# cure-lab/MagicDrive

Hardware: NVIDIA H100
Metric: 6-view 224x400 denoising-steps/sec (higher is better)
Workload: dtype bf16

## Files before the change

### magicdrive_b200/csrc/attention_wgmma.cuh

```cuda
#pragma once
#include "ptx.cuh"
#include "wgmma.cuh"

namespace mdb {

constexpr int ATT_BM = 128;

constexpr int ATT_MAX_SRC = 3;
struct AttnKvMaps {
  CUtensorMap k[ATT_MAX_SRC], v[ATT_MAX_SRC];
};

struct AttnParams {
  __nv_bfloat16* out;
  int ldo;
  int lq, lk;
  const int* kv_index;
  int n_sets;
  int n_src;
  float scale_log2;
  int q_step;
};

template <int D, int BN_ = 0>
struct AttnCfg {
  static constexpr int KD = (D + 63) / 64;
  static constexpr int D16 = (D + 15) / 16 * 16;
  static constexpr int BN = BN_ ? BN_ : ((D16 <= 64) ? 128 : 64);
  static constexpr int TILE_Q = ATT_BM * 128;
  static constexpr int TILE_KV = BN * 128;
  static constexpr int SMEM_Q = KD * TILE_Q;
  static constexpr int STAGES_FIT = (232448 - 1024 - 256 - SMEM_Q) / (2 * KD * TILE_KV);
  static constexpr int STAGES = STAGES_FIT > 4 ? 4 : STAGES_FIT;
  static constexpr int SMEM_KV = STAGES * 2 * KD * TILE_KV;
  static constexpr int kSmemBytes = SMEM_Q + SMEM_KV + 1024 + 256;
  static constexpr int kConsumerWarps = 8;
  static constexpr int kThreads = 32 * kConsumerWarps + 32;
  static constexpr int SACC = BN / 2;
  static constexpr int OACC = D16 / 2;
  static_assert(STAGES >= 1 && kSmemBytes <= 232448, "shared memory");
};

template <int D, int BN_>
__global__ void __launch_bounds__(AttnCfg<D, BN_>::kThreads, 1)
attention_wgmma_kernel(const __grid_constant__ CUtensorMap tmQ, const __grid_constant__ AttnKvMaps kvm, const AttnParams p) {
  using Cfg = AttnCfg<D, BN_>;
  constexpr int KD = Cfg::KD, D16 = Cfg::D16, BN = Cfg::BN, STAGES = Cfg::STAGES;
  constexpr int TILE_Q = Cfg::TILE_Q, TILE_KV = Cfg::TILE_KV;
  extern __shared__ uint8_t smem_raw[];
  uint8_t* smem = reinterpret_cast<uint8_t*>((reinterpret_cast<uintptr_t>(smem_raw) + 1023) & ~uintptr_t(1023));
  uint8_t* smQ = smem;
  uint8_t* smK = smQ + Cfg::SMEM_Q;
  uint8_t* smV = smK + STAGES * KD * TILE_KV;
  uint64_t* bars = reinterpret_cast<uint64_t*>(smV + STAGES * KD * TILE_KV);
  uint64_t* q_full = bars;
  uint64_t* q_empty = bars + 1;
  uint64_t* kv_full = bars + 2;
  uint64_t* kv_empty = bars + 2 + STAGES;

  const int warp = threadIdx.x >> 5, lane = threadIdx.x & 31;
  const int b = blockIdx.z, head = blockIdx.y;
  const int ntiles = (p.lk + BN - 1) / BN;
  const int nq = (p.lq + ATT_BM - 1) / ATT_BM;
  const int q_step = p.q_step > 0 ? p.q_step : nq;
  const int n_own = (nq - static_cast<int>(blockIdx.x) + q_step - 1) / q_step;
  const bool kv_resident = ntiles == 1 && p.n_sets == 1 && n_own > 1;
  auto q0_of = [&](int o) { return (static_cast<int>(blockIdx.x) + o * q_step) * ATT_BM; };

  if (warp == Cfg::kConsumerWarps && lane == 0) {
    prefetch_tmap(&tmQ);
    for (int i = 0; i < p.n_src; ++i) {
      prefetch_tmap(&kvm.k[i]);
      prefetch_tmap(&kvm.v[i]);
    }
    mbar_init(q_full, 1);
    mbar_init(q_empty, Cfg::kConsumerWarps);
    for (int i = 0; i < STAGES; ++i) {
      mbar_init(&kv_full[i], 1);
      mbar_init(&kv_empty[i], Cfg::kConsumerWarps);
    }
    fence_barrier_init();
  }
  __syncthreads();
  asm volatile("griddepcontrol.wait;" ::: "memory");
  asm volatile("griddepcontrol.launch_dependents;" ::: "memory");

  if (warp == Cfg::kConsumerWarps) {
    if (lane == 0) {
      int stage = 0;
      uint32_t phase = 0;
      for (int o = 0; o < n_own; ++o) {
        if (o > 0) mbar_wait(q_empty, static_cast<uint32_t>(o - 1) & 1u);
        mbar_arrive_expect_tx(q_full, KD * TILE_Q);
#pragma unroll
        for (int c = 0; c < KD; ++c) tma_load_4d(&tmQ, q_full, smQ + c * TILE_Q, c * 64, head, q0_of(o), b);
        if (kv_resident && o > 0) continue;
        for (int set = 0; set < p.n_sets; ++set) {
          const int kve = p.kv_index ? p.kv_index[b * p.n_sets + set] : b;
          const int kvb = kve & 0xffffff;
          const CUtensorMap* km = &kvm.k[kve >> 24];
          const CUtensorMap* vm = &kvm.v[kve >> 24];
          for (int j = 0; j < ntiles; ++j) {
            mbar_wait(&kv_empty[stage], phase ^ 1);
            mbar_arrive_expect_tx(&kv_full[stage], 2 * KD * TILE_KV);
#pragma unroll
            for (int c = 0; c < KD; ++c) {
              tma_load_4d(km, &kv_full[stage], smK + (stage * KD + c) * TILE_KV, c * 64, head, j * BN, kvb);
              tma_load_4d(vm, &kv_full[stage], smV + (stage * KD + c) * TILE_KV, c * 64, head, j * BN, kvb);
            }
            if (++stage == STAGES) {
              stage = 0;
              phase ^= 1;
            }
          }
        }
      }
    }
    return;
  }

  const int wg = warp >> 2;
  const int q = lane & 3;
  const int rloc = 64 * wg + 16 * (warp & 3) + (lane >> 2);
  const float sc = p.scale_log2;
  int stage = 0;
  uint32_t phase = 0;
  for (int o = 0; o < n_own; ++o) {
    const int q0 = q0_of(o);
    mbar_wait(q_full, static_cast<uint32_t>(o) & 1u);
    for (int set = 0; set < p.n_sets; ++set) {
      float oacc[Cfg::OACC];
#pragma unroll
      for (int i = 0; i < Cfg::OACC; ++i) oacc[i] = 0.f;
      float m[2] = {-INFINITY, -INFINITY}, l[2] = {0.f, 0.f};
      for (int j = 0; j < ntiles; ++j) {
        const int st = kv_resident ? 0 : stage;
        mbar_wait(&kv_full[st], kv_resident ? 0u : phase);
        float s[Cfg::SACC];
        wgmma_fence();
#pragma unroll
        for (int k = 0; k < D16 / 16; ++k) {
          const int c = k / 4, kk = k % 4;
          const uint64_t adesc = make_sw128_kmajor_desc(smem_u32(smQ + c * TILE_Q + wg * (64 * 128))) + 2 * kk;
          const uint64_t bdesc = make_sw128_kmajor_desc(smem_u32(smK + (st * KD + c) * TILE_KV)) + 2 * kk;
          WgmmaSS<BN>::run(s, adesc, bdesc, k > 0 ? 1u : 0u);
        }
        wgmma_commit();
        wgmma_wait<0>();
        const int kbase = j * BN;
        if (kbase + BN > p.lk) {
#pragma unroll
          for (int g = 0; g < BN / 8; ++g)
#pragma unroll
            for (int e = 0; e < 2; ++e)
              if (kbase + 8 * g + 2 * q + e >= p.lk) s[4 * g + e] = s[4 * g + 2 + e] = -INFINITY;
        }
        float corr[2];
#pragma unroll
        for (int h = 0; h < 2; ++h) {
          float mx = -INFINITY;
#pragma unroll
          for (int g = 0; g < BN / 8; ++g) mx = fmaxf(mx, fmaxf(s[4 * g + 2 * h], s[4 * g + 2 * h + 1]));
          mx = fmaxf(mx, __shfl_xor_sync(0xffffffffu, mx, 1));
          mx = fmaxf(mx, __shfl_xor_sync(0xffffffffu, mx, 2));
          const float m_new = fmaxf(m[h], mx * sc);
          corr[h] = exp2f(m[h] - m_new);
          m[h] = m_new;
        }
        uint32_t pa[BN / 16][4];
        float rs[2] = {0.f, 0.f};
#pragma unroll
        for (int kk = 0; kk < BN / 16; ++kk) {
#pragma unroll
          for (int r = 0; r < 4; ++r) {
            const int h = r & 1;
            const int i0 = 8 * kk + 4 * (r >> 1) + 2 * h;
            const float p0 = exp2f(fmaf(s[i0], sc, -m[h]));
            const float p1 = exp2f(fmaf(s[i0 + 1], sc, -m[h]));
            rs[h] += p0 + p1;
            pa[kk][r] = pack_bf16(p0, p1);
          }
        }
#pragma unroll
        for (int h = 0; h < 2; ++h) l[h] = l[h] * corr[h] + rs[h];
#pragma unroll
        for (int g = 0; g < D16 / 8; ++g) {
          oacc[4 * g] *= corr[0], oacc[4 * g + 1] *= corr[0];
          oacc[4 * g + 2] *= corr[1], oacc[4 * g + 3] *= corr[1];
        }
        wgmma_fence();
#pragma unroll
        for (int kk = 0; kk < BN / 16; ++kk) {
          const uint64_t bdesc = make_sw128_mnmajor_desc(smem_u32(smV + st * KD * TILE_KV), TILE_KV) + (2048u >> 4) * kk;
          WgmmaRSBmn<D16>::run(oacc, pa[kk], bdesc, 1u);
        }
        wgmma_commit();
        wgmma_wait<0>();
        if (!kv_resident) {
          if (lane == 0) mbar_arrive(&kv_empty[stage]);
          if (++stage == STAGES) {
            stage = 0;
            phase ^= 1;
          }
        }
      }
#pragma unroll
      for (int h = 0; h < 2; ++h) {
        l[h] += __shfl_xor_sync(0xffffffffu, l[h], 1);
        l[h] += __shfl_xor_sync(0xffffffffu, l[h], 2);
      }
      const float inv[2] = {1.0f / l[0], 1.0f / l[1]};
#pragma unroll
      for (int h = 0; h < 2; ++h) {
        const int qrow = q0 + rloc + 8 * h;
        if (qrow >= p.lq) continue;
        __nv_bfloat16* orow = p.out + (static_cast<long long>(b) * p.lq + qrow) * p.ldo + head * D;
#pragma unroll
        for (int g = 0; g < D16 / 8; ++g) {
          const int col = 8 * g + 2 * q;
          if (col >= D) continue;
          float f0 = oacc[4 * g + 2 * h] * inv[h], f1 = oacc[4 * g + 2 * h + 1] * inv[h];
          if (set > 0) {
            const float2 pf = __bfloat1622float2(*reinterpret_cast<const __nv_bfloat162*>(orow + col));
            f0 = __bfloat162float(__float2bfloat16_rn(f0)) + pf.x;
            f1 = __bfloat162float(__float2bfloat16_rn(f1)) + pf.y;
          }
          *reinterpret_cast<uint32_t*>(orow + col) = pack_bf16(f0, f1);
        }
      }
    }
    __syncwarp();
    if (lane == 0) mbar_arrive(q_empty);
  }
}

}
```

### magicdrive_b200/csrc/capi_attention.cu

```cuda
#include <cuda_bf16.h>
#include <cuda_runtime.h>

#include <stdlib.h>
#include <string.h>

#include "../../include/magicdrive_b200.h"
#define MDB_NEED_TENSORMAP
#include "common_host.h"
#include "attention_wgmma.cuh"

namespace {

bool make_qkv_map(CUtensorMap* m, const void* ptr, int d, int heads, int l, int b, int ld, int rows) {
  mdb::EncodeTiledFn enc = mdb::get_encode();
  if (!enc) return false;
  cuuint64_t dims[4] = {(cuuint64_t)d, (cuuint64_t)heads, (cuuint64_t)l, (cuuint64_t)b};
  cuuint64_t strides[3] = {(cuuint64_t)d * 2, (cuuint64_t)ld * 2, (cuuint64_t)l * ld * 2};
  cuuint32_t box[4] = {64u, 1u, (cuuint32_t)rows, 1u};
  cuuint32_t estr[4] = {1u, 1u, 1u, 1u};
  return enc(m, CU_TENSOR_MAP_DATA_TYPE_BFLOAT16, 4, const_cast<void*>(ptr), dims, strides, box, estr,
             CU_TENSOR_MAP_INTERLEAVE_NONE, CU_TENSOR_MAP_SWIZZLE_128B, CU_TENSOR_MAP_L2_PROMOTION_L2_256B,
             CU_TENSOR_MAP_FLOAT_OOB_FILL_NONE) == CUDA_SUCCESS;
}

struct KvSources {
  const void* k[mdb::ATT_MAX_SRC];
  const void* v[mdb::ATT_MAX_SRC];
  int ldk[mdb::ATT_MAX_SRC], ldv[mdb::ATT_MAX_SRC], b_kv[mdb::ATT_MAX_SRC];
  int n;
};

bool make_kv_maps(mdb::AttnKvMaps* m, const KvSources& s, int d, int heads, int lk, int rows) {
  for (int i = 0; i < mdb::ATT_MAX_SRC; ++i) {
    const int j = i < s.n ? i : 0;
    if (!make_qkv_map(&m->k[i], s.k[j], d, heads, lk, s.b_kv[j], s.ldk[j], rows) ||
        !make_qkv_map(&m->v[i], s.v[j], d, heads, lk, s.b_kv[j], s.ldv[j], rows))
      return false;
  }
  return true;
}

int attn_num_sms() {
  static int sms = 0;
  if (!sms) {
    int dev = 0;
    cudaGetDevice(&dev);
    if (cudaDeviceGetAttribute(&sms, cudaDevAttrMultiProcessorCount, dev) != cudaSuccess || sms <= 0) sms = 132;
  }
  return sms;
}

int multi_q_step(int b, int heads, int lq, int lk, int n_sets, int bn) {
  if (lk > bn || n_sets != 1) return 0;
  const char* e = getenv("MDB_ATTN_MULTIQ");
  if (e && e[0] == '0') return 0;
  const int nq = (lq + mdb::ATT_BM - 1) / mdb::ATT_BM;
  const long long per_tile_ctas = static_cast<long long>(b) * heads;
  const long long slots = attn_num_sms();
  if (per_tile_ctas * nq <= slots) return 0;
  long long gx = slots / per_tile_ctas;
  if (gx < 1) gx = 1;
  if (gx >= nq) return 0;
  return static_cast<int>(gx);
}

template <int D, int BN_>
int launch_attention(const void* q, int ldq, const KvSources& src, void* out, int ldo, int b, int heads, int lq, int lk,
                     const int* kv_index, int n_sets, float scale, cudaStream_t st) {
  using Cfg = mdb::AttnCfg<D, BN_>;
  static bool attr = false;
  if (!attr) {
    cudaError_t e = cudaFuncSetAttribute(mdb::attention_wgmma_kernel<D, BN_>, cudaFuncAttributeMaxDynamicSharedMemorySize, Cfg::kSmemBytes);
    if (e != cudaSuccess) return mdb::set_error(MDB_ERR_CUDA, "attention_wgmma_kernel smem attr: %s", cudaGetErrorString(e));
    attr = true;
  }
  CUtensorMap tq;
  mdb::AttnKvMaps kvm;
  if (!make_qkv_map(&tq, q, D, heads, lq, b, ldq, mdb::ATT_BM) || !make_kv_maps(&kvm, src, D, heads, lk, Cfg::BN))
    return mdb::set_error(MDB_ERR_CUDA, "mdb_attention: cuTensorMapEncodeTiled failed (d=%d heads=%d lq=%d lk=%d)", D, heads, lq, lk);
  mdb::AttnParams p;
  p.out = static_cast<__nv_bfloat16*>(out);
  p.ldo = ldo, p.lq = lq, p.lk = lk, p.kv_index = kv_index, p.n_sets = n_sets, p.n_src = src.n;
  p.scale_log2 = scale * 1.4426950408889634f;
  p.q_step = multi_q_step(b, heads, lq, lk, n_sets, Cfg::BN);
  dim3 grid(p.q_step > 0 ? p.q_step : (lq + mdb::ATT_BM - 1) / mdb::ATT_BM, heads, b);
  cudaError_t le = mdb::launch_pdl(mdb::attention_wgmma_kernel<D, BN_>, grid, dim3(Cfg::kThreads), Cfg::kSmemBytes, st, tq, kvm, p);
  if (le != cudaSuccess) return mdb::set_error(MDB_ERR_CUDA, "attention_wgmma_kernel launch: %s", cudaGetErrorString(le));
  cudaError_t e2 = cudaGetLastError();
  if (e2 != cudaSuccess) return mdb::set_error(MDB_ERR_CUDA, "attention_wgmma_kernel: %s", cudaGetErrorString(e2));
  return MDB_OK;
}

template <int BN_>
int attention_dispatch_bn(const void* q, int ldq, const KvSources& src, void* out, int ldo, int b, int heads, int lq, int lk, int d,
                          const int* kv_index, int n_sets, float scale, cudaStream_t st) {
  switch (d) {
    case 32: return launch_attention<32, BN_>(q, ldq, src, out, ldo, b, heads, lq, lk, kv_index, n_sets, scale, st);
    case 40: return launch_attention<40, BN_>(q, ldq, src, out, ldo, b, heads, lq, lk, kv_index, n_sets, scale, st);
    case 64: return launch_attention<64, BN_>(q, ldq, src, out, ldo, b, heads, lq, lk, kv_index, n_sets, scale, st);
    case 80: return launch_attention<80, BN_>(q, ldq, src, out, ldo, b, heads, lq, lk, kv_index, n_sets, scale, st);
    case 160: return launch_attention<160, BN_>(q, ldq, src, out, ldo, b, heads, lq, lk, kv_index, n_sets, scale, st);
    default: return mdb::set_error(MDB_ERR_UNSUPPORTED, "mdb_attention: head dim %d not instantiated (32, 40, 64, 80, 160)", d);
  }
}

int attention_dispatch(const void* q, int ldq, const KvSources& src, void* out, int ldo, int b, int heads, int lq, int lk, int d,
                       const int* kv_index, int n_sets, float scale, cudaStream_t st) {
  const char* e = getenv("MDB_ATTN_KERNEL");
  if (e && !strcmp(e, "tc2d")) return attention_dispatch_bn<64>(q, ldq, src, out, ldo, b, heads, lq, lk, d, kv_index, n_sets, scale, st);
  if (e && !strcmp(e, "tc")) return attention_dispatch_bn<128>(q, ldq, src, out, ldo, b, heads, lq, lk, d, kv_index, n_sets, scale, st);
  if (e && *e && strcmp(e, "tc2"))
    return mdb::set_error(MDB_ERR_INVALID, "mdb_attention: MDB_ATTN_KERNEL must be tc2, tc2d or tc (got %s)", e);
  return attention_dispatch_bn<0>(q, ldq, src, out, ldo, b, heads, lq, lk, d, kv_index, n_sets, scale, st);
}

}

extern "C" int mdb_attention_multi(const void* q, int ldq, int n_src, const void* const* k, const int* ldk, const void* const* v,
                                   const int* ldv, const int* b_kv, void* out, int ldo, int b, int heads, int lq, int lk, int d,
                                   const int* kv_index, int n_sets, float scale, void* stream) {
  using namespace mdb;
  if (!q || !k || !v || !ldk || !ldv || !b_kv || !out) return set_error(MDB_ERR_INVALID, "mdb_attention: null pointer");
  if (n_src < 1 || n_src > ATT_MAX_SRC) return set_error(MDB_ERR_INVALID, "mdb_attention: 1..%d K/V sources", ATT_MAX_SRC);
  if (n_sets < 1 || n_sets > 2 || (n_sets == 2 && !kv_index))
    return set_error(MDB_ERR_INVALID, "mdb_attention: n_sets must be 1 or 2 (2 needs kv_index)");
  if (scale <= 0.f) return set_error(MDB_ERR_INVALID, "mdb_attention: scale must be positive");
  if (lq <= 0 || lk <= 0 || b <= 0 || heads <= 0) return set_error(MDB_ERR_INVALID, "mdb_attention: bad shape");
  if (ldq % 8 || ldo % 8) return set_error(MDB_ERR_UNSUPPORTED, "mdb_attention: strides must be multiples of 8");
  KvSources src;
  src.n = n_src;
  for (int i = 0; i < n_src; ++i) {
    if (!k[i] || !v[i] || b_kv[i] <= 0) return set_error(MDB_ERR_INVALID, "mdb_attention: bad K/V source %d", i);
    if (ldk[i] % 8 || ldv[i] % 8) return set_error(MDB_ERR_UNSUPPORTED, "mdb_attention: strides must be multiples of 8");
    src.k[i] = k[i], src.v[i] = v[i], src.ldk[i] = ldk[i], src.ldv[i] = ldv[i], src.b_kv[i] = b_kv[i];
  }
  if (!kv_index && (n_src != 1 || b_kv[0] != b)) return set_error(MDB_ERR_INVALID, "mdb_attention: b_kv != b or several sources need kv_index");
  return attention_dispatch(q, ldq, src, out, ldo, b, heads, lq, lk, d, kv_index, n_sets, scale, static_cast<cudaStream_t>(stream));
}

extern "C" int mdb_attention(const void* q, int ldq, const void* k, int ldk, const void* v, int ldv, void* out, int ldo, int b,
                             int b_kv, int heads, int lq, int lk, int d, const int* kv_index, int n_sets, float scale,
                             void* stream) {
  return mdb_attention_multi(q, ldq, 1, &k, &ldk, &v, &ldv, &b_kv, out, ldo, b, heads, lq, lk, d, kv_index, n_sets, scale, stream);
}
```

### magicdrive_b200/csrc/ptx.cuh

```cuda
#pragma once
#include <cuda.h>
#include <cuda_bf16.h>
#include <cuda_runtime.h>
#include <stdint.h>

namespace mdb {

__device__ __forceinline__ uint32_t smem_u32(const void* p) {
  return static_cast<uint32_t>(__cvta_generic_to_shared(p));
}

__device__ __forceinline__ bool elect_one() {
  uint32_t pred = 0;
  asm volatile(
      "{\n\t"
      ".reg .pred P;\n\t"
      "elect.sync _|P, 0xffffffff;\n\t"
      "selp.b32 %0, 1, 0, P;\n\t"
      "}\n"
      : "=r"(pred));
  return pred != 0;
}

__device__ __forceinline__ void mbar_init(uint64_t* bar, uint32_t count) {
  asm volatile("mbarrier.init.shared::cta.b64 [%0], %1;" ::"r"(smem_u32(bar)), "r"(count));
}
__device__ __forceinline__ void fence_barrier_init() {
  asm volatile("fence.mbarrier_init.release.cluster;" ::: "memory");
}
__device__ __forceinline__ void fence_proxy_async() {
  asm volatile("fence.proxy.async.shared::cta;" ::: "memory");
}
__device__ __forceinline__ bool mbar_test(uint64_t* bar, uint32_t parity) {
  uint32_t ok;
  asm volatile(
      "{\n\t"
      ".reg .pred P1;\n\t"
      "mbarrier.test_wait.parity.shared::cta.b64 P1, [%1], %2;\n\t"
      "selp.u32 %0, 1, 0, P1;\n\t"
      "}\n"
      : "=r"(ok)
      : "r"(smem_u32(bar)), "r"(parity)
      : "memory");
  return ok != 0;
}
__device__ __forceinline__ void mbar_arrive_expect_tx(uint64_t* bar, uint32_t bytes) {
  asm volatile("mbarrier.arrive.expect_tx.shared::cta.b64 _, [%0], %1;" ::"r"(smem_u32(bar)), "r"(bytes)
               : "memory");
}
__device__ __forceinline__ void mbar_arrive(uint64_t* bar) {
  asm volatile("mbarrier.arrive.shared::cta.b64 _, [%0];" ::"r"(smem_u32(bar)) : "memory");
}
#ifndef MDB_MBAR_WAIT_MODE
#define MDB_MBAR_WAIT_MODE 0
#endif
__device__ __forceinline__ void mbar_wait(uint64_t* bar, uint32_t parity) {
#if MDB_MBAR_WAIT_MODE == 0
  asm volatile(
      "{\n\t"
      ".reg .pred P1;\n\t"
      "WAIT_LOOP:\n\t"
      "mbarrier.try_wait.parity.shared::cta.b64 P1, [%0], %1, 0x989680;\n\t"
      "@P1 bra DONE;\n\t"
      "bra WAIT_LOOP;\n\t"
      "DONE:\n\t"
      "}\n" ::"r"(smem_u32(bar)),
      "r"(parity)
      : "memory");
#elif MDB_MBAR_WAIT_MODE == 1
  asm volatile(
      "{\n\t"
      ".reg .pred P1;\n\t"
      "WAIT_LOOP:\n\t"
      "mbarrier.try_wait.parity.shared::cta.b64 P1, [%0], %1;\n\t"
      "@P1 bra DONE;\n\t"
      "bra WAIT_LOOP;\n\t"
      "DONE:\n\t"
      "}\n" ::"r"(smem_u32(bar)),
      "r"(parity)
      : "memory");
#else
  asm volatile(
      "{\n\t"
      ".reg .pred P1;\n\t"
      "WAIT_LOOP:\n\t"
      "mbarrier.test_wait.parity.shared::cta.b64 P1, [%0], %1;\n\t"
      "@P1 bra DONE;\n\t"
      "bra WAIT_LOOP;\n\t"
      "DONE:\n\t"
      "}\n" ::"r"(smem_u32(bar)),
      "r"(parity)
      : "memory");
#endif
}

__device__ __forceinline__ void prefetch_tmap(const CUtensorMap* m) {
  asm volatile("prefetch.tensormap [%0];" ::"l"(reinterpret_cast<uint64_t>(m)) : "memory");
}
__device__ __forceinline__ void tma_load_2d(const CUtensorMap* m, uint64_t* bar, void* dst, int c0, int c1) {
  asm volatile(
      "cp.async.bulk.tensor.2d.shared::cluster.global.mbarrier::complete_tx::bytes"
      " [%0], [%1, {%3, %4}], [%2];" ::"r"(smem_u32(dst)),
      "l"(reinterpret_cast<uint64_t>(m)), "r"(smem_u32(bar)), "r"(c0), "r"(c1)
      : "memory");
}
__device__ __forceinline__ void tma_load_4d(const CUtensorMap* m, uint64_t* bar, void* dst, int c0, int c1, int c2,
                                            int c3) {
  asm volatile(
      "cp.async.bulk.tensor.4d.shared::cluster.global.mbarrier::complete_tx::bytes"
      " [%0], [%1, {%3, %4, %5, %6}], [%2];" ::"r"(smem_u32(dst)),
      "l"(reinterpret_cast<uint64_t>(m)), "r"(smem_u32(bar)), "r"(c0), "r"(c1), "r"(c2), "r"(c3)
      : "memory");
}
__device__ __forceinline__ void tma_load_im2col_4d(const CUtensorMap* m, uint64_t* bar, void* dst, int c, int w, int h,
                                                   int n, uint16_t off_w, uint16_t off_h) {
  asm volatile(
      "cp.async.bulk.tensor.4d.shared::cluster.global.im2col.mbarrier::complete_tx::bytes"
      " [%0], [%1, {%3, %4, %5, %6}], [%2], {%7, %8};" ::"r"(smem_u32(dst)),
      "l"(reinterpret_cast<uint64_t>(m)), "r"(smem_u32(bar)), "r"(c), "r"(w), "r"(h), "r"(n), "h"(off_w), "h"(off_h)
      : "memory");
}

__device__ __forceinline__ uint64_t make_sw128_kmajor_desc(uint32_t smem_addr_bytes) {
  uint64_t d = 0;
  d |= static_cast<uint64_t>((smem_addr_bytes >> 4) & 0x3FFF);
  d |= static_cast<uint64_t>(1) << 16;
  d |= static_cast<uint64_t>((1024u >> 4) & 0x3FFF) << 32;
  d |= static_cast<uint64_t>(1) << 62;
  return d;
}
__device__ __forceinline__ uint64_t make_sw128_mnmajor_desc(uint32_t smem_addr_bytes, uint32_t lbo_bytes) {
  uint64_t d = 0;
  d |= static_cast<uint64_t>((smem_addr_bytes >> 4) & 0x3FFF);
  d |= static_cast<uint64_t>((lbo_bytes >> 4) & 0x3FFF) << 16;
  d |= static_cast<uint64_t>((1024u >> 4) & 0x3FFF) << 32;
  d |= static_cast<uint64_t>(1) << 62;
  return d;
}

__device__ __forceinline__ uint32_t pack_bf16(float a, float b) {
  __nv_bfloat162 h = __floats2bfloat162_rn(a, b);
  return *reinterpret_cast<uint32_t*>(&h);
}

}
```

### magicdrive_b200/csrc/wgmma.cuh

```cuda
#pragma once
#include <stdint.h>

namespace mdb {

__device__ __forceinline__ void wgmma_fence() { asm volatile("wgmma.fence.sync.aligned;" ::: "memory"); }
__device__ __forceinline__ void wgmma_commit() { asm volatile("wgmma.commit_group.sync.aligned;" ::: "memory"); }
template <int N>
__device__ __forceinline__ void wgmma_wait() {
  asm volatile("wgmma.wait_group.sync.aligned %0;" ::"n"(N) : "memory");
}

__device__ __forceinline__ void wgmma_ss_n64(float (&d)[32], uint64_t adesc, uint64_t bdesc, uint32_t accumulate) {
  asm volatile(
      "{\n\t.reg .pred p;\n\t"
      "setp.ne.b32 p, %34, 0;\n\t"
      "wgmma.mma_async.sync.aligned.m64n64k16.f32.bf16.bf16 "
      "{%0, %1, %2, %3, %4, %5, %6, %7, %8, %9, %10, %11, %12, %13, %14, %15, %16, %17, %18, %19, %20, %21, %22, %23, %24, %25, %26, %27, %28, %29, %30, %31}, "
      "%32, %33, p, 1, 1, 0, 0;\n\t}\n"
      : "+f"(d[0]), "+f"(d[1]), "+f"(d[2]), "+f"(d[3]), "+f"(d[4]), "+f"(d[5]), "+f"(d[6]), "+f"(d[7]), "+f"(d[8]), "+f"(d[9]), "+f"(d[10]), "+f"(d[11]), "+f"(d[12]), "+f"(d[13]), "+f"(d[14]), "+f"(d[15]), "+f"(d[16]), "+f"(d[17]), "+f"(d[18]), "+f"(d[19]), "+f"(d[20]), "+f"(d[21]), "+f"(d[22]), "+f"(d[23]), "+f"(d[24]), "+f"(d[25]), "+f"(d[26]), "+f"(d[27]), "+f"(d[28]), "+f"(d[29]), "+f"(d[30]), "+f"(d[31])
      : "l"(adesc), "l"(bdesc), "r"(accumulate));
}

__device__ __forceinline__ void wgmma_ss_n128(float (&d)[64], uint64_t adesc, uint64_t bdesc, uint32_t accumulate) {
  asm volatile(
      "{\n\t.reg .pred p;\n\t"
      "setp.ne.b32 p, %66, 0;\n\t"
      "wgmma.mma_async.sync.aligned.m64n128k16.f32.bf16.bf16 "
      "{%0, %1, %2, %3, %4, %5, %6, %7, %8, %9, %10, %11, %12, %13, %14, %15, %16, %17, %18, %19, %20, %21, %22, %23, %24, %25, %26, %27, %28, %29, %30, %31, %32, %33, %34, %35, %36, %37, %38, %39, %40, %41, %42, %43, %44, %45, %46, %47, %48, %49, %50, %51, %52, %53, %54, %55, %56, %57, %58, %59, %60, %61, %62, %63}, "
      "%64, %65, p, 1, 1, 0, 0;\n\t}\n"
      : "+f"(d[0]), "+f"(d[1]), "+f"(d[2]), "+f"(d[3]), "+f"(d[4]), "+f"(d[5]), "+f"(d[6]), "+f"(d[7]), "+f"(d[8]), "+f"(d[9]), "+f"(d[10]), "+f"(d[11]), "+f"(d[12]), "+f"(d[13]), "+f"(d[14]), "+f"(d[15]), "+f"(d[16]), "+f"(d[17]), "+f"(d[18]), "+f"(d[19]), "+f"(d[20]), "+f"(d[21]), "+f"(d[22]), "+f"(d[23]), "+f"(d[24]), "+f"(d[25]), "+f"(d[26]), "+f"(d[27]), "+f"(d[28]), "+f"(d[29]), "+f"(d[30]), "+f"(d[31]), "+f"(d[32]), "+f"(d[33]), "+f"(d[34]), "+f"(d[35]), "+f"(d[36]), "+f"(d[37]), "+f"(d[38]), "+f"(d[39]), "+f"(d[40]), "+f"(d[41]), "+f"(d[42]), "+f"(d[43]), "+f"(d[44]), "+f"(d[45]), "+f"(d[46]), "+f"(d[47]), "+f"(d[48]), "+f"(d[49]), "+f"(d[50]), "+f"(d[51]), "+f"(d[52]), "+f"(d[53]), "+f"(d[54]), "+f"(d[55]), "+f"(d[56]), "+f"(d[57]), "+f"(d[58]), "+f"(d[59]), "+f"(d[60]), "+f"(d[61]), "+f"(d[62]), "+f"(d[63])
      : "l"(adesc), "l"(bdesc), "r"(accumulate));
}

__device__ __forceinline__ void wgmma_ss_n160(float (&d)[80], uint64_t adesc, uint64_t bdesc, uint32_t accumulate) {
  asm volatile(
      "{\n\t.reg .pred p;\n\t"
      "setp.ne.b32 p, %82, 0;\n\t"
      "wgmma.mma_async.sync.aligned.m64n160k16.f32.bf16.bf16 "
      "{%0, %1, %2, %3, %4, %5, %6, %7, %8, %9, %10, %11, %12, %13, %14, %15, %16, %17, %18, %19, %20, %21, %22, %23, %24, %25, %26, %27, %28, %29, %30, %31, %32, %33, %34, %35, %36, %37, %38, %39, %40, %41, %42, %43, %44, %45, %46, %47, %48, %49, %50, %51, %52, %53, %54, %55, %56, %57, %58, %59, %60, %61, %62, %63, %64, %65, %66, %67, %68, %69, %70, %71, %72, %73, %74, %75, %76, %77, %78, %79}, "
      "%80, %81, p, 1, 1, 0, 0;\n\t}\n"
      : "+f"(d[0]), "+f"(d[1]), "+f"(d[2]), "+f"(d[3]), "+f"(d[4]), "+f"(d[5]), "+f"(d[6]), "+f"(d[7]), "+f"(d[8]), "+f"(d[9]), "+f"(d[10]), "+f"(d[11]), "+f"(d[12]), "+f"(d[13]), "+f"(d[14]), "+f"(d[15]), "+f"(d[16]), "+f"(d[17]), "+f"(d[18]), "+f"(d[19]), "+f"(d[20]), "+f"(d[21]), "+f"(d[22]), "+f"(d[23]), "+f"(d[24]), "+f"(d[25]), "+f"(d[26]), "+f"(d[27]), "+f"(d[28]), "+f"(d[29]), "+f"(d[30]), "+f"(d[31]), "+f"(d[32]), "+f"(d[33]), "+f"(d[34]), "+f"(d[35]), "+f"(d[36]), "+f"(d[37]), "+f"(d[38]), "+f"(d[39]), "+f"(d[40]), "+f"(d[41]), "+f"(d[42]), "+f"(d[43]), "+f"(d[44]), "+f"(d[45]), "+f"(d[46]), "+f"(d[47]), "+f"(d[48]), "+f"(d[49]), "+f"(d[50]), "+f"(d[51]), "+f"(d[52]), "+f"(d[53]), "+f"(d[54]), "+f"(d[55]), "+f"(d[56]), "+f"(d[57]), "+f"(d[58]), "+f"(d[59]), "+f"(d[60]), "+f"(d[61]), "+f"(d[62]), "+f"(d[63]), "+f"(d[64]), "+f"(d[65]), "+f"(d[66]), "+f"(d[67]), "+f"(d[68]), "+f"(d[69]), "+f"(d[70]), "+f"(d[71]), "+f"(d[72]), "+f"(d[73]), "+f"(d[74]), "+f"(d[75]), "+f"(d[76]), "+f"(d[77]), "+f"(d[78]), "+f"(d[79])
      : "l"(adesc), "l"(bdesc), "r"(accumulate));
}

__device__ __forceinline__ void wgmma_ss_n256(float (&d)[128], uint64_t adesc, uint64_t bdesc, uint32_t accumulate) {
  asm volatile(
      "{\n\t.reg .pred p;\n\t"
      "setp.ne.b32 p, %130, 0;\n\t"
      "wgmma.mma_async.sync.aligned.m64n256k16.f32.bf16.bf16 "
      "{%0, %1, %2, %3, %4, %5, %6, %7, %8, %9, %10, %11, %12, %13, %14, %15, %16, %17, %18, %19, %20, %21, %22, %23, %24, %25, %26, %27, %28, %29, %30, %31, %32, %33, %34, %35, %36, %37, %38, %39, %40, %41, %42, %43, %44, %45, %46, %47, %48, %49, %50, %51, %52, %53, %54, %55, %56, %57, %58, %59, %60, %61, %62, %63, %64, %65, %66, %67, %68, %69, %70, %71, %72, %73, %74, %75, %76, %77, %78, %79, %80, %81, %82, %83, %84, %85, %86, %87, %88, %89, %90, %91, %92, %93, %94, %95, %96, %97, %98, %99, %100, %101, %102, %103, %104, %105, %106, %107, %108, %109, %110, %111, %112, %113, %114, %115, %116, %117, %118, %119, %120, %121, %122, %123, %124, %125, %126, %127}, "
      "%128, %129, p, 1, 1, 0, 0;\n\t}\n"
      : "+f"(d[0]), "+f"(d[1]), "+f"(d[2]), "+f"(d[3]), "+f"(d[4]), "+f"(d[5]), "+f"(d[6]), "+f"(d[7]), "+f"(d[8]), "+f"(d[9]), "+f"(d[10]), "+f"(d[11]), "+f"(d[12]), "+f"(d[13]), "+f"(d[14]), "+f"(d[15]), "+f"(d[16]), "+f"(d[17]), "+f"(d[18]), "+f"(d[19]), "+f"(d[20]), "+f"(d[21]), "+f"(d[22]), "+f"(d[23]), "+f"(d[24]), "+f"(d[25]), "+f"(d[26]), "+f"(d[27]), "+f"(d[28]), "+f"(d[29]), "+f"(d[30]), "+f"(d[31]), "+f"(d[32]), "+f"(d[33]), "+f"(d[34]), "+f"(d[35]), "+f"(d[36]), "+f"(d[37]), "+f"(d[38]), "+f"(d[39]), "+f"(d[40]), "+f"(d[41]), "+f"(d[42]), "+f"(d[43]), "+f"(d[44]), "+f"(d[45]), "+f"(d[46]), "+f"(d[47]), "+f"(d[48]), "+f"(d[49]), "+f"(d[50]), "+f"(d[51]), "+f"(d[52]), "+f"(d[53]), "+f"(d[54]), "+f"(d[55]), "+f"(d[56]), "+f"(d[57]), "+f"(d[58]), "+f"(d[59]), "+f"(d[60]), "+f"(d[61]), "+f"(d[62]), "+f"(d[63]), "+f"(d[64]), "+f"(d[65]), "+f"(d[66]), "+f"(d[67]), "+f"(d[68]), "+f"(d[69]), "+f"(d[70]), "+f"(d[71]), "+f"(d[72]), "+f"(d[73]), "+f"(d[74]), "+f"(d[75]), "+f"(d[76]), "+f"(d[77]), "+f"(d[78]), "+f"(d[79]), "+f"(d[80]), "+f"(d[81]), "+f"(d[82]), "+f"(d[83]), "+f"(d[84]), "+f"(d[85]), "+f"(d[86]), "+f"(d[87]), "+f"(d[88]), "+f"(d[89]), "+f"(d[90]), "+f"(d[91]), "+f"(d[92]), "+f"(d[93]), "+f"(d[94]), "+f"(d[95]), "+f"(d[96]), "+f"(d[97]), "+f"(d[98]), "+f"(d[99]), "+f"(d[100]), "+f"(d[101]), "+f"(d[102]), "+f"(d[103]), "+f"(d[104]), "+f"(d[105]), "+f"(d[106]), "+f"(d[107]), "+f"(d[108]), "+f"(d[109]), "+f"(d[110]), "+f"(d[111]), "+f"(d[112]), "+f"(d[113]), "+f"(d[114]), "+f"(d[115]), "+f"(d[116]), "+f"(d[117]), "+f"(d[118]), "+f"(d[119]), "+f"(d[120]), "+f"(d[121]), "+f"(d[122]), "+f"(d[123]), "+f"(d[124]), "+f"(d[125]), "+f"(d[126]), "+f"(d[127])
      : "l"(adesc), "l"(bdesc), "r"(accumulate));
}

__device__ __forceinline__ void wgmma_rs_n32_bmn(float (&d)[16], const uint32_t (&a)[4], uint64_t bdesc, uint32_t accumulate) {
  asm volatile(
      "{\n\t.reg .pred p;\n\t"
      "setp.ne.b32 p, %21, 0;\n\t"
      "wgmma.mma_async.sync.aligned.m64n32k16.f32.bf16.bf16 "
      "{%0, %1, %2, %3, %4, %5, %6, %7, %8, %9, %10, %11, %12, %13, %14, %15}, "
      "{%16, %17, %18, %19}, %20, p, 1, 1, 1;\n\t}\n"
      : "+f"(d[0]), "+f"(d[1]), "+f"(d[2]), "+f"(d[3]), "+f"(d[4]), "+f"(d[5]), "+f"(d[6]), "+f"(d[7]), "+f"(d[8]), "+f"(d[9]), "+f"(d[10]), "+f"(d[11]), "+f"(d[12]), "+f"(d[13]), "+f"(d[14]), "+f"(d[15])
      : "r"(a[0]), "r"(a[1]), "r"(a[2]), "r"(a[3]), "l"(bdesc), "r"(accumulate));
}

__device__ __forceinline__ void wgmma_rs_n48_bmn(float (&d)[24], const uint32_t (&a)[4], uint64_t bdesc, uint32_t accumulate) {
  asm volatile(
      "{\n\t.reg .pred p;\n\t"
      "setp.ne.b32 p, %29, 0;\n\t"
      "wgmma.mma_async.sync.aligned.m64n48k16.f32.bf16.bf16 "
      "{%0, %1, %2, %3, %4, %5, %6, %7, %8, %9, %10, %11, %12, %13, %14, %15, %16, %17, %18, %19, %20, %21, %22, %23}, "
      "{%24, %25, %26, %27}, %28, p, 1, 1, 1;\n\t}\n"
      : "+f"(d[0]), "+f"(d[1]), "+f"(d[2]), "+f"(d[3]), "+f"(d[4]), "+f"(d[5]), "+f"(d[6]), "+f"(d[7]), "+f"(d[8]), "+f"(d[9]), "+f"(d[10]), "+f"(d[11]), "+f"(d[12]), "+f"(d[13]), "+f"(d[14]), "+f"(d[15]), "+f"(d[16]), "+f"(d[17]), "+f"(d[18]), "+f"(d[19]), "+f"(d[20]), "+f"(d[21]), "+f"(d[22]), "+f"(d[23])
      : "r"(a[0]), "r"(a[1]), "r"(a[2]), "r"(a[3]), "l"(bdesc), "r"(accumulate));
}

__device__ __forceinline__ void wgmma_rs_n64_bmn(float (&d)[32], const uint32_t (&a)[4], uint64_t bdesc, uint32_t accumulate) {
  asm volatile(
      "{\n\t.reg .pred p;\n\t"
      "setp.ne.b32 p, %37, 0;\n\t"
      "wgmma.mma_async.sync.aligned.m64n64k16.f32.bf16.bf16 "
      "{%0, %1, %2, %3, %4, %5, %6, %7, %8, %9, %10, %11, %12, %13, %14, %15, %16, %17, %18, %19, %20, %21, %22, %23, %24, %25, %26, %27, %28, %29, %30, %31}, "
      "{%32, %33, %34, %35}, %36, p, 1, 1, 1;\n\t}\n"
      : "+f"(d[0]), "+f"(d[1]), "+f"(d[2]), "+f"(d[3]), "+f"(d[4]), "+f"(d[5]), "+f"(d[6]), "+f"(d[7]), "+f"(d[8]), "+f"(d[9]), "+f"(d[10]), "+f"(d[11]), "+f"(d[12]), "+f"(d[13]), "+f"(d[14]), "+f"(d[15]), "+f"(d[16]), "+f"(d[17]), "+f"(d[18]), "+f"(d[19]), "+f"(d[20]), "+f"(d[21]), "+f"(d[22]), "+f"(d[23]), "+f"(d[24]), "+f"(d[25]), "+f"(d[26]), "+f"(d[27]), "+f"(d[28]), "+f"(d[29]), "+f"(d[30]), "+f"(d[31])
      : "r"(a[0]), "r"(a[1]), "r"(a[2]), "r"(a[3]), "l"(bdesc), "r"(accumulate));
}

__device__ __forceinline__ void wgmma_rs_n80_bmn(float (&d)[40], const uint32_t (&a)[4], uint64_t bdesc, uint32_t accumulate) {
  asm volatile(
      "{\n\t.reg .pred p;\n\t"
      "setp.ne.b32 p, %45, 0;\n\t"
      "wgmma.mma_async.sync.aligned.m64n80k16.f32.bf16.bf16 "
      "{%0, %1, %2, %3, %4, %5, %6, %7, %8, %9, %10, %11, %12, %13, %14, %15, %16, %17, %18, %19, %20, %21, %22, %23, %24, %25, %26, %27, %28, %29, %30, %31, %32, %33, %34, %35, %36, %37, %38, %39}, "
      "{%40, %41, %42, %43}, %44, p, 1, 1, 1;\n\t}\n"
      : "+f"(d[0]), "+f"(d[1]), "+f"(d[2]), "+f"(d[3]), "+f"(d[4]), "+f"(d[5]), "+f"(d[6]), "+f"(d[7]), "+f"(d[8]), "+f"(d[9]), "+f"(d[10]), "+f"(d[11]), "+f"(d[12]), "+f"(d[13]), "+f"(d[14]), "+f"(d[15]), "+f"(d[16]), "+f"(d[17]), "+f"(d[18]), "+f"(d[19]), "+f"(d[20]), "+f"(d[21]), "+f"(d[22]), "+f"(d[23]), "+f"(d[24]), "+f"(d[25]), "+f"(d[26]), "+f"(d[27]), "+f"(d[28]), "+f"(d[29]), "+f"(d[30]), "+f"(d[31]), "+f"(d[32]), "+f"(d[33]), "+f"(d[34]), "+f"(d[35]), "+f"(d[36]), "+f"(d[37]), "+f"(d[38]), "+f"(d[39])
      : "r"(a[0]), "r"(a[1]), "r"(a[2]), "r"(a[3]), "l"(bdesc), "r"(accumulate));
}

__device__ __forceinline__ void wgmma_rs_n160_bmn(float (&d)[80], const uint32_t (&a)[4], uint64_t bdesc, uint32_t accumulate) {
  asm volatile(
      "{\n\t.reg .pred p;\n\t"
      "setp.ne.b32 p, %85, 0;\n\t"
      "wgmma.mma_async.sync.aligned.m64n160k16.f32.bf16.bf16 "
      "{%0, %1, %2, %3, %4, %5, %6, %7, %8, %9, %10, %11, %12, %13, %14, %15, %16, %17, %18, %19, %20, %21, %22, %23, %24, %25, %26, %27, %28, %29, %30, %31, %32, %33, %34, %35, %36, %37, %38, %39, %40, %41, %42, %43, %44, %45, %46, %47, %48, %49, %50, %51, %52, %53, %54, %55, %56, %57, %58, %59, %60, %61, %62, %63, %64, %65, %66, %67, %68, %69, %70, %71, %72, %73, %74, %75, %76, %77, %78, %79}, "
      "{%80, %81, %82, %83}, %84, p, 1, 1, 1;\n\t}\n"
      : "+f"(d[0]), "+f"(d[1]), "+f"(d[2]), "+f"(d[3]), "+f"(d[4]), "+f"(d[5]), "+f"(d[6]), "+f"(d[7]), "+f"(d[8]), "+f"(d[9]), "+f"(d[10]), "+f"(d[11]), "+f"(d[12]), "+f"(d[13]), "+f"(d[14]), "+f"(d[15]), "+f"(d[16]), "+f"(d[17]), "+f"(d[18]), "+f"(d[19]), "+f"(d[20]), "+f"(d[21]), "+f"(d[22]), "+f"(d[23]), "+f"(d[24]), "+f"(d[25]), "+f"(d[26]), "+f"(d[27]), "+f"(d[28]), "+f"(d[29]), "+f"(d[30]), "+f"(d[31]), "+f"(d[32]), "+f"(d[33]), "+f"(d[34]), "+f"(d[35]), "+f"(d[36]), "+f"(d[37]), "+f"(d[38]), "+f"(d[39]), "+f"(d[40]), "+f"(d[41]), "+f"(d[42]), "+f"(d[43]), "+f"(d[44]), "+f"(d[45]), "+f"(d[46]), "+f"(d[47]), "+f"(d[48]), "+f"(d[49]), "+f"(d[50]), "+f"(d[51]), "+f"(d[52]), "+f"(d[53]), "+f"(d[54]), "+f"(d[55]), "+f"(d[56]), "+f"(d[57]), "+f"(d[58]), "+f"(d[59]), "+f"(d[60]), "+f"(d[61]), "+f"(d[62]), "+f"(d[63]), "+f"(d[64]), "+f"(d[65]), "+f"(d[66]), "+f"(d[67]), "+f"(d[68]), "+f"(d[69]), "+f"(d[70]), "+f"(d[71]), "+f"(d[72]), "+f"(d[73]), "+f"(d[74]), "+f"(d[75]), "+f"(d[76]), "+f"(d[77]), "+f"(d[78]), "+f"(d[79])
      : "r"(a[0]), "r"(a[1]), "r"(a[2]), "r"(a[3]), "l"(bdesc), "r"(accumulate));
}

template <int N> struct WgmmaSS;
template <> struct WgmmaSS<64> { static __device__ __forceinline__ void run(float (&d)[32], uint64_t a, uint64_t b, uint32_t acc) { wgmma_ss_n64(d, a, b, acc); } };
template <> struct WgmmaSS<128> { static __device__ __forceinline__ void run(float (&d)[64], uint64_t a, uint64_t b, uint32_t acc) { wgmma_ss_n128(d, a, b, acc); } };
template <> struct WgmmaSS<160> { static __device__ __forceinline__ void run(float (&d)[80], uint64_t a, uint64_t b, uint32_t acc) { wgmma_ss_n160(d, a, b, acc); } };
template <> struct WgmmaSS<256> { static __device__ __forceinline__ void run(float (&d)[128], uint64_t a, uint64_t b, uint32_t acc) { wgmma_ss_n256(d, a, b, acc); } };
template <int N> struct WgmmaRSBmn;
template <> struct WgmmaRSBmn<32> { static __device__ __forceinline__ void run(float (&d)[16], const uint32_t (&a)[4], uint64_t b, uint32_t acc) { wgmma_rs_n32_bmn(d, a, b, acc); } };
template <> struct WgmmaRSBmn<48> { static __device__ __forceinline__ void run(float (&d)[24], const uint32_t (&a)[4], uint64_t b, uint32_t acc) { wgmma_rs_n48_bmn(d, a, b, acc); } };
template <> struct WgmmaRSBmn<64> { static __device__ __forceinline__ void run(float (&d)[32], const uint32_t (&a)[4], uint64_t b, uint32_t acc) { wgmma_rs_n64_bmn(d, a, b, acc); } };
template <> struct WgmmaRSBmn<80> { static __device__ __forceinline__ void run(float (&d)[40], const uint32_t (&a)[4], uint64_t b, uint32_t acc) { wgmma_rs_n80_bmn(d, a, b, acc); } };
template <> struct WgmmaRSBmn<160> { static __device__ __forceinline__ void run(float (&d)[80], const uint32_t (&a)[4], uint64_t b, uint32_t acc) { wgmma_rs_n160_bmn(d, a, b, acc); } };

}
```

Measured before the change: 48.72.

## Pipeline FlashAttention with warpgroup ping-pong, split K/V barriers and persistent grid

Restructures the wgmma attention kernel into a FA3-style schedule. The next tile's QK^T is issued alongside the previous tile's PV, and named barriers alternate the two consumer warpgroups so softmax overlaps tensor-core work. K and V get separate full/empty barriers, and registers are rebalanced with setmaxnreg using a 128-thread producer warpgroup. The grid becomes persistent, with work items over (batch, head, q-tile) split contiguously per SM so K/V can stay resident across consecutive q-tiles. This adds complexity and risks deadlock or load imbalance in exchange for overlapping softmax with MMA and cutting tail effects.

```diff
diff --git a/magicdrive_b200/csrc/attention_wgmma.cuh b/magicdrive_b200/csrc/attention_wgmma.cuh
--- a/magicdrive_b200/csrc/attention_wgmma.cuh
+++ b/magicdrive_b200/csrc/attention_wgmma.cuh
@@ -15,11 +15,12 @@
   __nv_bfloat16* out;
   int ldo;
   int lq, lk;
+  int b, heads;
   const int* kv_index;
   int n_sets;
   int n_src;
   float scale_log2;
-  int q_step;
+  int kv_reuse;
 };
 
 template <int D, int BN_ = 0>
@@ -35,7 +36,9 @@
   static constexpr int SMEM_KV = STAGES * 2 * KD * TILE_KV;
   static constexpr int kSmemBytes = SMEM_Q + SMEM_KV + 1024 + 256;
   static constexpr int kConsumerWarps = 8;
-  static constexpr int kThreads = 32 * kConsumerWarps + 32;
+  static constexpr int kConsumers = 32 * kConsumerWarps;
+  static constexpr int kThreads = kConsumers + 128;
+  static constexpr int kProducerRegs = 40, kConsumerRegs = 232;
   static constexpr int SACC = BN / 2;
   static constexpr int OACC = D16 / 2;
   static_assert(STAGES >= 1 && kSmemBytes <= 232448, "shared memory");
@@ -55,19 +58,22 @@
   uint64_t* bars = reinterpret_cast<uint64_t*>(smV + STAGES * KD * TILE_KV);
   uint64_t* q_full = bars;
   uint64_t* q_empty = bars + 1;
-  uint64_t* kv_full = bars + 2;
-  uint64_t* kv_empty = bars + 2 + STAGES;
-
-  const int warp = threadIdx.x >> 5, lane = threadIdx.x & 31;
-  const int b = blockIdx.z, head = blockIdx.y;
+  uint64_t* k_full = bars + 2;
+  uint64_t* k_empty = k_full + STAGES;
+  uint64_t* v_full = k_empty + STAGES;
+  uint64_t* v_empty = v_full + STAGES;
+
+  const int tid = threadIdx.x;
   const int ntiles = (p.lk + BN - 1) / BN;
   const int nq = (p.lq + ATT_BM - 1) / ATT_BM;
-  const int q_step = p.q_step > 0 ? p.q_step : nq;
-  const int n_own = (nq - static_cast<int>(blockIdx.x) + q_step - 1) / q_step;
-  const bool kv_resident = ntiles == 1 && p.n_sets == 1 && n_own > 1;
-  auto q0_of = [&](int o) { return (static_cast<int>(blockIdx.x) + o * q_step) * ATT_BM; };
-
-  if (warp == Cfg::kConsumerWarps && lane == 0) {
+  const int n_items = nq * p.heads * p.b;
+  const bool single_kv = ntiles == 1 && p.n_sets == 1;
+  const int first = single_kv ? static_cast<int>(static_cast<long long>(blockIdx.x) * n_items / gridDim.x) : blockIdx.x;
+  const int last = single_kv ? static_cast<int>(static_cast<long long>(blockIdx.x + 1) * n_items / gridDim.x) : n_items;
+  const int step = single_kv ? 1 : gridDim.x;
+  auto reuses_kv = [&](int it) { return p.kv_reuse && single_kv && it > first && it < last && it / nq == (it - 1) / nq; };
+
+  if (tid == Cfg::kConsumers) {
     prefetch_tmap(&tmQ);
     for (int i = 0; i < p.n_src; ++i) {
       prefetch_tmap(&kvm.k[i]);
@@ -76,8 +82,10 @@
     mbar_init(q_full, 1);
     mbar_init(q_empty, Cfg::kConsumerWarps);
     for (int i = 0; i < STAGES; ++i) {
-      mbar_init(&kv_full[i], 1);
-      mbar_init(&kv_empty[i], Cfg::kConsumerWarps);
+      mbar_init(&k_full[i], 1);
+      mbar_init(&k_empty[i], Cfg::kConsumerWarps);
+      mbar_init(&v_full[i], 1);
+      mbar_init(&v_empty[i], Cfg::kConsumerWarps);
     }
     fence_barrier_init();
   }
@@ -85,29 +93,33 @@
   asm volatile("griddepcontrol.wait;" ::: "memory");
   asm volatile("griddepcontrol.launch_dependents;" ::: "memory");
 
-  if (warp == Cfg::kConsumerWarps) {
-    if (lane == 0) {
+  if (tid >= Cfg::kConsumers) {
+    setmaxnreg_dec<Cfg::kProducerRegs>();
+    if (tid == Cfg::kConsumers) {
       int stage = 0;
       uint32_t phase = 0;
-      for (int o = 0; o < n_own; ++o) {
-        if (o > 0) mbar_wait(q_empty, static_cast<uint32_t>(o - 1) & 1u);
+      uint32_t n_done = 0;
+      for (int it = first; it < last; it += step, ++n_done) {
+        const int bh = it / nq, head = bh % p.heads, b = bh / p.heads;
+        if (n_done > 0) mbar_wait(q_empty, (n_done - 1) & 1u);
         mbar_arrive_expect_tx(q_full, KD * TILE_Q);
 #pragma unroll
-        for (int c = 0; c < KD; ++c) tma_load_4d(&tmQ, q_full, smQ + c * TILE_Q, c * 64, head, q0_of(o), b);
-        if (kv_resident && o > 0) continue;
+        for (int c = 0; c < KD; ++c) tma_load_4d(&tmQ, q_full, smQ + c * TILE_Q, c * 64, head, (it % nq) * ATT_BM, b);
+        if (reuses_kv(it)) continue;
         for (int set = 0; set < p.n_sets; ++set) {
           const int kve = p.kv_index ? p.kv_index[b * p.n_sets + set] : b;
           const int kvb = kve & 0xffffff;
           const CUtensorMap* km = &kvm.k[kve >> 24];
           const CUtensorMap* vm = &kvm.v[kve >> 24];
           for (int j = 0; j < ntiles; ++j) {
-            mbar_wait(&kv_empty[stage], phase ^ 1);
-            mbar_arrive_expect_tx(&kv_full[stage], 2 * KD * TILE_KV);
-#pragma unroll
-            for (int c = 0; c < KD; ++c) {
-              tma_load_4d(km, &kv_full[stage], smK + (stage * KD + c) * TILE_KV, c * 64, head, j * BN, kvb);
-              tma_load_4d(vm, &kv_full[stage], smV + (stage * KD + c) * TILE_KV, c * 64, head, j * BN, kvb);
-            }
+            mbar_wait(&k_empty[stage], phase ^ 1);
+            mbar_arrive_expect_tx(&k_full[stage], KD * TILE_KV);
+#pragma unroll
+            for (int c = 0; c < KD; ++c) tma_load_4d(km, &k_full[stage], smK + (stage * KD + c) * TILE_KV, c * 64, head, j * BN, kvb);
+            mbar_wait(&v_empty[stage], phase ^ 1);
+            mbar_arrive_expect_tx(&v_full[stage], KD * TILE_KV);
+#pragma unroll
+            for (int c = 0; c < KD; ++c) tma_load_4d(vm, &v_full[stage], smV + (stage * KD + c) * TILE_KV, c * 64, head, j * BN, kvb);
             if (++stage == STAGES) {
               stage = 0;
               phase ^= 1;
@@ -119,34 +131,67 @@
     return;
   }
 
+  setmaxnreg_inc<Cfg::kConsumerRegs>();
+  const int warp = tid >> 5, lane = tid & 31;
   const int wg = warp >> 2;
   const int q = lane & 3;
   const int rloc = 64 * wg + 16 * (warp & 3) + (lane >> 2);
   const float sc = p.scale_log2;
-  int stage = 0;
-  uint32_t phase = 0;
-  for (int o = 0; o < n_own; ++o) {
-    const int q0 = q0_of(o);
-    mbar_wait(q_full, static_cast<uint32_t>(o) & 1u);
+  const uint32_t bar_own = 1 + wg, bar_other = 2 - wg;
+  if (wg == 0) named_bar_arrive(bar_own, Cfg::kConsumers);
+  int ks = 0, vs = 0;
+  uint32_t kph = 0, vph = 0;
+  auto release = [&](uint64_t* empty, int& st, uint32_t& ph) {
+    if (lane == 0) mbar_arrive(&empty[st]);
+    if (++st == STAGES) {
+      st = 0;
+      ph ^= 1;
+    }
+  };
+  uint32_t n_done = 0;
+  for (int it = first; it < last; it += step, ++n_done) {
+    const int bh = it / nq, head = bh % p.heads, b = bh / p.heads;
+    const int q0 = (it % nq) * ATT_BM;
+    const bool keep_kv = reuses_kv(it + 1);
+    mbar_wait(q_full, n_done & 1u);
     for (int set = 0; set < p.n_sets; ++set) {
+      const bool last_set = set == p.n_sets - 1;
       float oacc[Cfg::OACC];
 #pragma unroll
       for (int i = 0; i < Cfg::OACC; ++i) oacc[i] = 0.f;
-      float m[2] = {-INFINITY, -INFINITY}, l[2] = {0.f, 0.f};
-      for (int j = 0; j < ntiles; ++j) {
-        const int st = kv_resident ? 0 : stage;
-        mbar_wait(&kv_full[st], kv_resident ? 0u : phase);
-        float s[Cfg::SACC];
-        wgmma_fence();
+      float m[2] = {-INFINITY, -INFINITY}, l[2] = {0.f, 0.f}, corr[2];
+      float s[Cfg::SACC];
+      uint32_t pa[BN / 16][4];
+      auto issue_qk = [&]() {
 #pragma unroll
         for (int k = 0; k < D16 / 16; ++k) {
           const int c = k / 4, kk = k % 4;
           const uint64_t adesc = make_sw128_kmajor_desc(smem_u32(smQ + c * TILE_Q + wg * (64 * 128))) + 2 * kk;
-          const uint64_t bdesc = make_sw128_kmajor_desc(smem_u32(smK + (st * KD + c) * TILE_KV)) + 2 * kk;
+          const uint64_t bdesc = make_sw128_kmajor_desc(smem_u32(smK + (ks * KD + c) * TILE_KV)) + 2 * kk;
           WgmmaSS<BN>::run(s, adesc, bdesc, k > 0 ? 1u : 0u);
         }
         wgmma_commit();
-        wgmma_wait<0>();
+      };
+      auto issue_pv = [&]() {
+#pragma unroll
+        for (int kk = 0; kk < BN / 16; ++kk) {
+          const uint64_t bdesc = make_sw128_mnmajor_desc(smem_u32(smV + vs * KD * TILE_KV), TILE_KV) + (2048u >> 4) * kk;
+          WgmmaRSBmn<D16>::run(oacc, pa[kk], bdesc, 1u);
+        }
+        wgmma_commit();
+      };
+      auto rescale_o = [&]() {
+#pragma unroll
+        for (int g = 0; g < D16 / 8; ++g) {
+          oacc[4 * g] *= corr[0], oacc[4 * g + 1] *= corr[0];
+          oacc[4 * g + 2] *= corr[1], oacc[4 * g + 3] *= corr[1];
+        }
+      };
+      auto softmax = [&](int j) {
+#pragma unroll
+        for (int i = 0; i < Cfg::SACC; ++i) wgmma_fence_operand(s[i]);
+        if (last_set && j == ntiles - 1 && lane == 0) mbar_arrive(q_empty);
+        if (!keep_kv) release(k_empty, ks, kph);
         const int kbase = j * BN;
         if (kbase + BN > p.lk) {
 #pragma unroll
@@ -155,7 +200,6 @@
             for (int e = 0; e < 2; ++e)
               if (kbase + 8 * g + 2 * q + e >= p.lk) s[4 * g + e] = s[4 * g + 2 + e] = -INFINITY;
         }
-        float corr[2];
 #pragma unroll
         for (int h = 0; h < 2; ++h) {
           float mx = -INFINITY;
@@ -167,7 +211,6 @@
           corr[h] = exp2f(m[h] - m_new);
           m[h] = m_new;
         }
-        uint32_t pa[BN / 16][4];
         float rs[2] = {0.f, 0.f};
 #pragma unroll
         for (int kk = 0; kk < BN / 16; ++kk) {
@@ -178,32 +221,56 @@
             const float p0 = exp2f(fmaf(s[i0], sc, -m[h]));
             const float p1 = exp2f(fmaf(s[i0 + 1], sc, -m[h]));
             rs[h] += p0 + p1;
-            pa[kk][r] = pack_bf16(p0, p1);
+            s[i0] = p0, s[i0 + 1] = p1;
           }
         }
 #pragma unroll
         for (int h = 0; h < 2; ++h) l[h] = l[h] * corr[h] + rs[h];
-#pragma unroll
-        for (int g = 0; g < D16 / 8; ++g) {
-          oacc[4 * g] *= corr[0], oacc[4 * g + 1] *= corr[0];
-          oacc[4 * g + 2] *= corr[1], oacc[4 * g + 3] *= corr[1];
-        }
+      };
+      auto pack_p = [&]() {
+#pragma unroll
+        for (int kk = 0; kk < BN / 16; ++kk)
+#pragma unroll
+          for (int r = 0; r < 4; ++r) {
+            const int i0 = 8 * kk + 4 * (r >> 1) + 2 * (r & 1);
+            pa[kk][r] = pack_bf16(s[i0], s[i0 + 1]);
+          }
+      };
+      auto pv_retired = [&]() {
+        wgmma_wait<0>();
+#pragma unroll
+        for (int i = 0; i < Cfg::OACC; ++i) wgmma_fence_operand(oacc[i]);
+      };
+
+      mbar_wait(&k_full[ks], kph);
+      named_bar_sync(bar_own, Cfg::kConsumers);
+      wgmma_fence();
+      issue_qk();
+      named_bar_arrive(bar_other, Cfg::kConsumers);
+      wgmma_wait<0>();
+      softmax(0);
+      pack_p();
+      for (int j = 1; j < ntiles; ++j) {
+        rescale_o();
+        mbar_wait(&v_full[vs], vph);
+        mbar_wait(&k_full[ks], kph);
+        named_bar_sync(bar_own, Cfg::kConsumers);
         wgmma_fence();
-#pragma unroll
-        for (int kk = 0; kk < BN / 16; ++kk) {
-          const uint64_t bdesc = make_sw128_mnmajor_desc(smem_u32(smV + st * KD * TILE_KV), TILE_KV) + (2048u >> 4) * kk;
-          WgmmaRSBmn<D16>::run(oacc, pa[kk], bdesc, 1u);
-        }
-        wgmma_commit();
-        wgmma_wait<0>();
-        if (!kv_resident) {
-          if (lane == 0) mbar_arrive(&kv_empty[stage]);
-          if (++stage == STAGES) {
-            stage = 0;
-            phase ^= 1;
-          }
-        }
+        issue_qk();
+        issue_pv();
+        named_bar_arrive(bar_other, Cfg::kConsumers);
+        wgmma_wait<1>();
+        softmax(j);
+        pv_retired();
+        release(v_empty, vs, vph);
+        pack_p();
       }
+      rescale_o();
+      mbar_wait(&v_full[vs], vph);
+      wgmma_fence();
+      issue_pv();
+      pv_retired();
+      if (!keep_kv) release(v_empty, vs, vph);
 #pragma unroll
       for (int h = 0; h < 2; ++h) {
         l[h] += __shfl_xor_sync(0xffffffffu, l[h], 1);
@@ -229,9 +296,8 @@
         }
       }
     }
-    __syncwarp();
-    if (lane == 0) mbar_arrive(q_empty);
   }
+  if (wg == 0) named_bar_sync(bar_own, Cfg::kConsumers);
 }
 
 }
diff --git a/magicdrive_b200/csrc/capi_attention.cu b/magicdrive_b200/csrc/capi_attention.cu
--- a/magicdrive_b200/csrc/capi_attention.cu
+++ b/magicdrive_b200/csrc/capi_attention.cu
@@ -1,6 +1,7 @@
 #include <cuda_bf16.h>
 #include <cuda_runtime.h>
 
+#include <limits.h>
 #include <stdlib.h>
 #include <string.h>
 
@@ -50,18 +51,10 @@
   return sms;
 }
 
-int multi_q_step(int b, int heads, int lq, int lk, int n_sets, int bn) {
+int multi_q(int lk, int n_sets, int bn) {
   if (lk > bn || n_sets != 1) return 0;
   const char* e = getenv("MDB_ATTN_MULTIQ");
-  if (e && e[0] == '0') return 0;
-  const int nq = (lq + mdb::ATT_BM - 1) / mdb::ATT_BM;
-  const long long per_tile_ctas = static_cast<long long>(b) * heads;
-  const long long slots = attn_num_sms();
-  if (per_tile_ctas * nq <= slots) return 0;
-  long long gx = slots / per_tile_ctas;
-  if (gx < 1) gx = 1;
-  if (gx >= nq) return 0;
-  return static_cast<int>(gx);
+  return e && e[0] == '0' ? 0 : 1;
 }
 
 template <int D, int BN_>
@@ -80,10 +73,12 @@
     return mdb::set_error(MDB_ERR_CUDA, "mdb_attention: cuTensorMapEncodeTiled failed (d=%d heads=%d lq=%d lk=%d)", D, heads, lq, lk);
   mdb::AttnParams p;
   p.out = static_cast<__nv_bfloat16*>(out);
-  p.ldo = ldo, p.lq = lq, p.lk = lk, p.kv_index = kv_index, p.n_sets = n_sets, p.n_src = src.n;
+  p.ldo = ldo, p.lq = lq, p.lk = lk, p.b = b, p.heads = heads, p.kv_index = kv_index, p.n_sets = n_sets, p.n_src = src.n;
   p.scale_log2 = scale * 1.4426950408889634f;
-  p.q_step = multi_q_step(b, heads, lq, lk, n_sets, Cfg::BN);
-  dim3 grid(p.q_step > 0 ? p.q_step : (lq + mdb::ATT_BM - 1) / mdb::ATT_BM, heads, b);
+  p.kv_reuse = multi_q(lk, n_sets, Cfg::BN);
+  const long long items = static_cast<long long>((lq + mdb::ATT_BM - 1) / mdb::ATT_BM) * heads * b;
+  if (items > INT_MAX) return mdb::set_error(MDB_ERR_UNSUPPORTED, "mdb_attention: %lld work items", items);
+  dim3 grid(static_cast<unsigned>(items < attn_num_sms() ? items : attn_num_sms()));
   cudaError_t le = mdb::launch_pdl(mdb::attention_wgmma_kernel<D, BN_>, grid, dim3(Cfg::kThreads), Cfg::kSmemBytes, st, tq, kvm, p);
   if (le != cudaSuccess) return mdb::set_error(MDB_ERR_CUDA, "attention_wgmma_kernel launch: %s", cudaGetErrorString(le));
   cudaError_t e2 = cudaGetLastError();
diff --git a/magicdrive_b200/csrc/ptx.cuh b/magicdrive_b200/csrc/ptx.cuh
--- a/magicdrive_b200/csrc/ptx.cuh
+++ b/magicdrive_b200/csrc/ptx.cuh
@@ -94,6 +94,21 @@
 #endif
 }
 
+__device__ __forceinline__ void named_bar_sync(uint32_t id, uint32_t threads) {
+  asm volatile("bar.sync %0, %1;" ::"r"(id), "r"(threads) : "memory");
+}
+__device__ __forceinline__ void named_bar_arrive(uint32_t id, uint32_t threads) {
+  asm volatile("bar.arrive %0, %1;" ::"r"(id), "r"(threads) : "memory");
+}
+template <int N>
+__device__ __forceinline__ void setmaxnreg_dec() {
+  asm volatile("setmaxnreg.dec.sync.aligned.u32 %0;" ::"n"(N));
+}
+template <int N>
+__device__ __forceinline__ void setmaxnreg_inc() {
+  asm volatile("setmaxnreg.inc.sync.aligned.u32 %0;" ::"n"(N));
+}
+
 __device__ __forceinline__ void prefetch_tmap(const CUtensorMap* m) {
   asm volatile("prefetch.tensormap [%0];" ::"l"(reinterpret_cast<uint64_t>(m)) : "memory");
 }
diff --git a/magicdrive_b200/csrc/wgmma.cuh b/magicdrive_b200/csrc/wgmma.cuh
--- a/magicdrive_b200/csrc/wgmma.cuh
+++ b/magicdrive_b200/csrc/wgmma.cuh
@@ -9,6 +9,7 @@
 __device__ __forceinline__ void wgmma_wait() {
   asm volatile("wgmma.wait_group.sync.aligned %0;" ::"n"(N) : "memory");
 }
+__device__ __forceinline__ void wgmma_fence_operand(float& r) { asm volatile("" : "+f"(r)::"memory"); }
 
 __device__ __forceinline__ void wgmma_ss_n64(float (&d)[32], uint64_t adesc, uint64_t bdesc, uint32_t accumulate) {
   asm volatile(
```

After: 49.43 (median of 6 runs). No clear change (+1.5%).
